# yunjinli/visual-slam

Measured on AMD Instinct MI355X. Metric: stereo frames/sec, detect+describe (1500 feats) + stereo match, 752x480, higher is better.
Workload: dtype u8/f32/f64; 1 GPU; synthetic 752x480 stereo, 1500 feats/frame (BASELINE configs[1]); independent streams per GPU (configs[3]); inputs_resident_in_hbm=True, distinct_stereo_pairs_per_gpu=1024, distinct_scenes_per_gpu=64, stereo_frames_per_pass_per_gpu=1024, hip_streams=2, stereo_frames_per_launch=512, num_features=1500, match=threshold 70, ratio 1.2, cross-check

## Files before the change

include/vslam_hip.h:

```cpp
#ifndef VSLAM_HIP_H
#define VSLAM_HIP_H

#include <stddef.h>
#include <stdint.h>

#ifdef __cplusplus
extern "C" {
#endif

#define VSL_OK 0
#define VSL_ERR_INVALID (-1)
#define VSL_ERR_HIP (-2)
#define VSL_ERR_NOMEM (-3)
#define VSL_ERR_CAPACITY (-4)
#define VSL_ERR_NO_DEVICE (-5)
#define VSL_ERR_IO (-6)
#define VSL_ERR_NUMERIC (-7)

typedef struct vsl_ctx vsl_ctx;


const char* vsl_version(void);
const char* vsl_last_error(const vsl_ctx* ctx);
int vsl_device_count(void);
// ... 74 lines not shown
int vsl_frames_upload(vsl_ctx* ctx, vsl_frames* f, int first, int n, const uint8_t* imgs,
                      size_t pitch, size_t img_stride);
int vsl_host_register(vsl_ctx* ctx, void* ptr, size_t bytes);
int vsl_host_unregister(vsl_ctx* ctx, void* ptr);
int vsl_frames_detect_describe(vsl_ctx* ctx, vsl_frames* f, int first, int n, int num_features,
                               int rotate_features);
int vsl_frames_resolve_ties(vsl_ctx* ctx, vsl_frames* f, int* n_resolved);
int vsl_frames_exact_fallbacks(const vsl_frames* f);
int vsl_ctx_set_tie_eps(vsl_ctx* ctx, double eps);
int vsl_ctx_set_diagnostic(vsl_ctx* ctx, const char* name, int value);
int vsl_ctx_get_diagnostic(vsl_ctx* ctx, const char* name, int* value);

int vsl_frames_match(vsl_ctx* ctx, vsl_frames* f, const int32_t* slot_pairs, int n_pairs,
                     int threshold, double dist_2_best);
int vsl_frames_download_keypoints(vsl_ctx* ctx, vsl_frames* f, int slot, int cap,
                                  double* corners_xy, double* angles, uint64_t* desc, int* n_out);
int vsl_frames_download_matches(vsl_ctx* ctx, vsl_frames* f, int pair, int cap_pairs,
                                int32_t* pairs, int* n_out);
int vsl_frames_download_counts(vsl_ctx* ctx, vsl_frames* f, int n_images, int32_t* n_keypoints,
                               int n_pairs, int32_t* n_matches);

int vsl_frames_stereo_inliers(vsl_ctx* ctx, vsl_frames* f, int first_pair, int n_pairs, int model_a, const double* intr8_a,
                              int model_b, const double* intr8_b, const double* E9, const double* R9_0_1,
                              const double* t3_0_1, double threshold, int triangulate);
int vsl_frames_download_inliers(vsl_ctx* ctx, vsl_frames* f, int pair, int cap_pairs, int32_t* pairs, double* points_c,
                                int* n_out);
int vsl_frames_download_inlier_counts(vsl_ctx* ctx, vsl_frames* f, int n_pairs, int32_t* counts);
int vsl_find_inliers_essential(vsl_ctx* ctx, int model_a, const double* intr8_a, int model_b, const double* intr8_b,
                               const double* E9, const double* kp_a_xy, int n_a, const double* kp_b_xy, int n_b,
                               const int32_t* matches, int n_matches, double threshold, const double* R9_0_1,
                               const double* t3_0_1, int32_t* pairs_out, double* points_out, int* n_out);

int vsl_frames_download_candidate_counts(vsl_ctx* ctx, vsl_frames* f, int n_images, int32_t* n_candidates);

int vsl_diag_sqrt_check(vsl_ctx* ctx, uint32_t lo_bits, uint32_t hi_bits, unsigned long long* n_mismatch);

int vsl_diag_frames_describe_at(vsl_ctx* ctx, vsl_frames* f, int first, int n, const int32_t* corners_xy,
                                const int32_t* counts, int cap, int rotate_features, int32_t* moments,
                                int32_t* tie_rec, int tie_rec_cap, int* n_ties);

int vsl_diag_frames_set_keypoints(vsl_ctx* ctx, vsl_frames* f, int first, int n, const int32_t* counts, int cap,
                                  const int32_t* corners_xy, const uint64_t* desc);

int vsl_map_create(vsl_ctx* ctx, int cap_landmarks, int cap_descriptors, vsl_map** out);
void vsl_map_destroy(vsl_map* map);
int vsl_map_append_descriptors(vsl_map* map, int n, const uint64_t* desc, int* first_index);
int vsl_map_append_descriptors_from_frame(vsl_map* map, vsl_frames* f, int slot, int n, const int32_t* feature_ids,
                                          int* first_index);
int vsl_map_set_landmarks(vsl_map* map, int n, const double* points, const int32_t* obs_start,
                          const int32_t* obs_pool_index);
int vsl_map_info(const vsl_map* map, int* n_landmarks, int* n_observation_refs, int* n_descriptors);
int vsl_map_track(vsl_map* map, vsl_frames* f, int slot, const double* pose7, int cam_model, const double* intr8, int width,
                  int height, double cam_z_threshold, double match_max_dist_2d, int feature_match_threshold,
                  double feature_match_dist_2_best, int32_t* pairs, int* n_pairs, int* n_projected);
int vsl_map_track_corners(vsl_map* map, vsl_frames* f, int slot, const double* pose7, int cam_model, const double* intr8,
                          int width, int height, double cam_z_threshold, double match_max_dist_2d, int feature_match_threshold,
                          double feature_match_dist_2_best, int32_t* pairs, int* n_pairs, int* n_projected, double* corners_xy,
                          int* n_corners);

enum { VSL_CAM_DS = 0, VSL_CAM_PINHOLE = 1, VSL_CAM_EUCM = 2, VSL_CAM_KB4 = 3 };

typedef struct vsl_ba_problem {
  int32_t n_cams;
  int32_t n_lms;
  int32_t n_obs;
  int32_t cam_model[2];
// ... 173 lines not shown
```

visual-slam_amd/__init__.py:

```python
import ctypes as C
import os
from pathlib import Path

import numpy as np

_DIR = Path(__file__).resolve().parent
_SO = _DIR / "libvslam_hip.so"
_LIB = None

u8p = C.POINTER(C.c_uint8)
i32p = C.POINTER(C.c_int32)
u32p = C.POINTER(C.c_uint32)
u64p = C.POINTER(C.c_uint64)
i64p = C.POINTER(C.c_int64)
f32p = C.POINTER(C.c_float)
f64p = C.POINTER(C.c_double)

STAGES = ["response", "select", "describe", "match", "match_finalize", "ba_linearize", "ba_schur",
          "ba_solve", "bow_transform", "bow_score", "ba_finish", "ba_step"]

SPD_PATHS = ["none", "dense_panels", "band_panels", "band_fused", "band_two_ended", "bcr", "bcr_cyclic"]

OK = 0
CAM_DS, CAM_PINHOLE, CAM_EUCM, CAM_KB4 = 0, 1, 2, 3
# ... 953 lines not shown

    def bow_vectors(self, first, n, voc, num_features=1500, levelsup=4, db=None, cap_per_image=None, host_outputs=True):
        L, ctx = self.ctx.L, self.ctx
        n = int(n)
        cap = (2 * num_features + 512 if cap_per_image is None else int(cap_per_image)) if host_outputs else 0
        nfeat = np.zeros(max(n, 1), np.int32)
        index = np.zeros(max(n, 1), np.int32)
        for attempt in range(2):
            m = max(n * cap, 1)
            ids, vals = np.zeros(m, np.uint32), np.zeros(m, np.float64)
            fn, ff = np.zeros(m, np.uint32), np.zeros(m, np.uint32)
            nnz, fvn = np.zeros(max(n, 1), np.int32), np.zeros(max(n, 1), np.int32)
            rc = L.vsl_frames_bow_vectors(ctx.h, self.h, int(first), n, voc.h if voc is not None else None, int(num_features),
                                          int(levelsup), db.h if db is not None else None, index.ctypes.data_as(i32p), cap,
                                          ids.ctypes.data_as(u32p), vals.ctypes.data_as(f64p), nnz.ctypes.data_as(i32p),
                                          fn.ctypes.data_as(u32p), ff.ctypes.data_as(u32p), fvn.ctypes.data_as(i32p),
                                          nfeat.ctypes.data_as(i32p))
            if rc != -4 or cap == 0 or cap_per_image is not None or nfeat[:n].max(initial=0) <= cap:
                break
            cap = int(nfeat[:n].max())
        ctx._ck(rc)
        out = None
        if host_outputs:
            out = [(ids[i * cap:i * cap + nnz[i]].copy(), vals[i * cap:i * cap + nnz[i]].copy(),
                    fn[i * cap:i * cap + fvn[i]].copy(), ff[i * cap:i * cap + fvn[i]].copy()) for i in range(n)]
        return (out, index[:n].copy()) if db is not None else out

    def candidate_counts(self, n_images):
        nc = np.zeros(max(n_images, 1), np.int32)
        self.ctx._ck(self.ctx.L.vsl_frames_download_candidate_counts(self.ctx.h, self.h, int(n_images),
                                                                     nc.ctypes.data_as(i32p)))
        return nc[:n_images].copy()

    def counts(self, n_images, n_pairs):
        nk = np.zeros(max(n_images, 1), np.int32)
        nm = np.zeros(max(n_pairs, 1), np.int32)
        self.ctx._ck(self.ctx.L.vsl_frames_download_counts(self.ctx.h, self.h, int(n_images),
                                                           nk.ctypes.data_as(i32p), int(n_pairs),
                                                           nm.ctypes.data_as(i32p)))
        return nk[:n_images].copy(), nm[:n_pairs].copy()


class Map:

    def __init__(self, ctx, cap_landmarks=4096, cap_descriptors=16384):
        self.ctx = ctx
        hnd = C.c_void_p()
        ctx._ck(ctx.L.vsl_map_create(ctx.h, int(cap_landmarks), int(cap_descriptors), C.byref(hnd)))
        self.h = hnd

    def close(self):
        if getattr(self, "h", None):
            self.ctx.L.vsl_map_destroy(self.h)
            self.h = None

    def __del__(self):
        try:
            self.close()
        except Exception:
            pass

    def append_descriptors(self, desc):
        desc = np.ascontiguousarray(desc, np.uint64).reshape(-1, 4)
        first = C.c_int32()
        self.ctx._ck(self.ctx.L.vsl_map_append_descriptors(self.h, len(desc), desc.ctypes.data_as(u64p), C.byref(first)))
        return first.value
# ... 41 lines not shown
```

visual-slam_amd/csrc/ctx.hip:

```cpp
#include <cmath>

#include "vsl_common.h"

static thread_local char g_noctx_err[512] = "";

int vsl_fail(vsl_ctx* ctx, int code, const char* fmt, ...) {
  char* dst = ctx ? ctx->err : g_noctx_err;
  va_list ap;
  va_start(ap, fmt);
  vsnprintf(dst, 512, fmt, ap);
  va_end(ap);
  return code;
}

extern "C" const char* vsl_version(void) { return "vslam_hip 0.1 (gfx950)"; }

extern "C" const char* vsl_last_error(const vsl_ctx* ctx) { return ctx ? ctx->err : g_noctx_err; }

extern "C" int vsl_device_count(void) {
  int n = 0;
  if (hipGetDeviceCount(&n) != hipSuccess) return 0;
  return n;
}

// ... 204 lines not shown
    ctx->stage_launches[i] = 0;
  }
  return rc;
}

template <class T>
static hipError_t dalloc(T** p, size_t n) {
  return hipMalloc((void**)p, n * sizeof(T));
}

int vsl_frames_alloc(vsl_ctx* ctx, int max_images, int w, int h, int F, int max_pairs, vsl_frames** out) {
  if (!ctx || !out) return VSL_ERR_INVALID;
  *out = nullptr;
  if (max_images <= 0 || w < 40 || h < 40 || w > 65535 || h > 65535 || F <= 0 || max_pairs < 0 || (int64_t)w * h >= (1ll << 31) ||
      F >= (1 << 22))
    return vsl_fail(ctx, VSL_ERR_INVALID, "vsl_frames_create: bad sizes images=%d w=%d h=%d F=%d pairs=%d", max_images, w, h, F, max_pairs);
  VSL_HIP(ctx, hipSetDevice(ctx->device));
  vsl_frames* f = new (std::nothrow) vsl_frames;
  if (!f) return vsl_fail(ctx, VSL_ERR_NOMEM, "out of host memory");
  f->device = ctx->device;
  f->max_images = max_images;
  f->w = w;
  f->h = h;
  f->F = F;
  f->max_pairs = max_pairs;
  f->cand_cap = (size_t)w * h;
  f->tie_cap = 4096;
  const size_t px = (size_t)w * h, M = (size_t)max_images, P = (size_t)(max_pairs > 0 ? max_pairs : 1);
  bool ok = true;
  ok = ok && dalloc(&f->images, M * px) == hipSuccess;
  ok = ok && dalloc(&f->response, M * px) == hipSuccess;
  ok = ok && dalloc(&f->meta, M * VSL_META_STRIDE) == hipSuccess;
  ok = ok && dalloc(&f->cand, M * f->cand_cap) == hipSuccess;
  ok = ok && dalloc(&f->kp_xy, M * F * 2) == hipSuccess;
  ok = ok && dalloc(&f->kp_count, M) == hipSuccess;
  ok = ok && dalloc(&f->kp_moments, M * F * 2) == hipSuccess;
  ok = ok && dalloc(&f->kp_angle, M * F) == hipSuccess;
  ok = ok && dalloc(&f->kp_desc, M * F * 4) == hipSuccess;
  ok = ok && dalloc(&f->pair_slots, P * 2) == hipSuccess;
  ok = ok && dalloc(&f->best_key, P * 2 * F) == hipSuccess;
  ok = ok && dalloc(&f->second_key, P * 2 * F) == hipSuccess;
  ok = ok && dalloc(&f->matches, P * F * 2) == hipSuccess;
  ok = ok && dalloc(&f->match_count, P) == hipSuccess;
  ok = ok && dalloc(&f->exact_list, M * VSL_EXACT_CAP) == hipSuccess;
  const int tiles_x = (w + (1 << VSL_TILE_LX) - 1) >> VSL_TILE_LX, tiles_y = (h + (1 << VSL_TILE_LY) - 1) >> VSL_TILE_LY;
  if (w % 16 == 0 && F < (1 << (32 - VSL_TILE_LX - VSL_TILE_LY)) && tiles_x * tiles_y <= 1024) {
    f->tiles_x = tiles_x;
    f->tiles = tiles_x * tiles_y;
    ok = ok && dalloc(&f->tile_off, M * (size_t)(f->tiles + 1)) == hipSuccess;
    ok = ok && dalloc(&f->tile_ent, M * F) == hipSuccess;
  }
  ok = ok && dalloc(&f->tie_count, 1) == hipSuccess;
  ok = ok && dalloc(&f->tie_rec, (size_t)f->tie_cap * 4) == hipSuccess;
  if (!ok) {
    vsl_frames_destroy(f);
    return vsl_fail(ctx, VSL_ERR_NOMEM, "device allocation failed for frame store (%d images %dx%d)", max_images, w, h);
  }
  (void)hipMemsetAsync(f->kp_count, 0, M * sizeof(int32_t), ctx->stream);
  (void)hipMemsetAsync(f->match_count, 0, P * sizeof(int32_t), ctx->stream);
  (void)hipMemsetAsync(f->tie_count, 0, sizeof(int32_t), ctx->stream);
  (void)hipMemsetAsync(f->meta, 0, M * VSL_META_STRIDE * sizeof(int32_t), ctx->stream);
  VSL_HIP(ctx, hipStreamSynchronize(ctx->stream));
  *out = f;
  return VSL_OK;
}

extern "C" int vsl_frames_create(vsl_ctx* ctx, int max_images, int w, int h, int max_features, int max_pairs,
                                 vsl_frames** out) {
  return vsl_frames_alloc(ctx, max_images, w, h, max_features, max_pairs, out);
}

extern "C" int vsl_frames_destroy(vsl_frames* f) {
  if (!f) return VSL_OK;
  (void)hipSetDevice(f->device);
  (void)hipDeviceSynchronize();
  void* ptrs[] = {f->images, f->response, f->meta, f->cand, f->kp_xy, f->kp_count,
                  f->kp_moments, f->kp_angle, f->kp_desc, f->pair_slots, f->best_key, f->second_key,
                  f->matches, f->match_count, f->tie_count, f->tie_rec, f->sel_grid, f->exact_list, f->tile_off, f->tile_ent,
                  f->st_pairs, f->st_points, f->st_count};
  for (void* p : ptrs)
    if (p) (void)hipFree(p);
  delete f;
  return VSL_OK;
}

extern "C" void* vsl_frames_images_dev(vsl_frames* f) { return f ? (void*)f->images : nullptr; }

extern "C" int vsl_frames_upload(vsl_ctx* ctx, vsl_frames* f, int first, int n, const uint8_t* imgs, size_t pitch,
                                 size_t img_stride) {
  if (!ctx || !f || !imgs || first < 0 || n < 0 || first + n > f->max_images || pitch < (size_t)f->w)
    return vsl_fail(ctx, VSL_ERR_INVALID, "vsl_frames_upload: bad arguments");
  if (n == 0) return VSL_OK;
  VSL_HIP(ctx, hipSetDevice(ctx->device));
  const size_t img_bytes = (size_t)f->w * f->h;
  if (pitch == (size_t)f->w && img_stride == img_bytes) {
    VSL_HIP(ctx, hipMemcpyAsync(f->images + (size_t)first * img_bytes, imgs, (size_t)n * img_bytes, hipMemcpyHostToDevice,
                                ctx->stream));
    return VSL_OK;
  }
  for (int i = 0; i < n; i++) {
    VSL_HIP(ctx, hipMemcpy2DAsync(f->images + (size_t)(first + i) * img_bytes, f->w, imgs + (size_t)i * img_stride,
                                  pitch, f->w, f->h, hipMemcpyHostToDevice, ctx->stream));
  }
  return VSL_OK;
}

extern "C" int vsl_host_register(vsl_ctx* ctx, void* ptr, size_t bytes) {
  if (!ctx || !ptr || bytes == 0) return vsl_fail(ctx, VSL_ERR_INVALID, "vsl_host_register: bad arguments");
  VSL_HIP(ctx, hipSetDevice(ctx->device));
  VSL_HIP(ctx, hipHostRegister(ptr, bytes, hipHostRegisterDefault));
  return VSL_OK;
// ... 58 lines not shown
    ctx->scratch = nullptr;
  }
  if (!ctx->scratch) {
    int rc = vsl_frames_alloc(ctx, 2, w, h, feat, 1, &ctx->scratch);
    if (rc) return rc;
    ctx->scratch_w = w;
    ctx->scratch_h = h;
    ctx->scratch_feat = feat;
  }
  *out = ctx->scratch;
  return VSL_OK;
}

extern "C" int vsl_frames_download_counts(vsl_ctx* ctx, vsl_frames* f, int n_images, int32_t* n_keypoints,
                                          int n_pairs, int32_t* n_matches) {
  if (!ctx || !f || n_images < 0 || n_images > f->max_images || n_pairs < 0 || n_pairs > f->max_pairs)
    return vsl_fail(ctx, VSL_ERR_INVALID, "vsl_frames_download_counts: bad arguments");
  if (n_images > 0 && n_keypoints)
    VSL_HIP(ctx, hipMemcpyAsync(n_keypoints, f->kp_count, sizeof(int32_t) * n_images, hipMemcpyDeviceToHost, ctx->stream));
  if (n_pairs > 0 && n_matches)
    VSL_HIP(ctx, hipMemcpyAsync(n_matches, f->match_count, sizeof(int32_t) * n_pairs, hipMemcpyDeviceToHost, ctx->stream));
  VSL_HIP(ctx, hipStreamSynchronize(ctx->stream));
  return VSL_OK;
}

extern "C" int vsl_frames_download_candidate_counts(vsl_ctx* ctx, vsl_frames* f, int n_images, int32_t* n_candidates) {
  if (!ctx || !f || n_images < 0 || n_images > f->max_images || !n_candidates)
    return vsl_fail(ctx, VSL_ERR_INVALID, "vsl_frames_download_candidate_counts: bad arguments");
  if (n_images == 0) return VSL_OK;
  std::vector<int32_t> m((size_t)n_images * VSL_META_STRIDE);
  VSL_HIP(ctx, hipMemcpyAsync(m.data(), f->meta, sizeof(int32_t) * m.size(), hipMemcpyDeviceToHost, ctx->stream));
  VSL_HIP(ctx, hipStreamSynchronize(ctx->stream));
  for (int i = 0; i < n_images; i++) n_candidates[i] = m[(size_t)i * VSL_META_STRIDE + VSL_META_NCAND_LAST];
  return VSL_OK;
}

extern "C" int vsl_frames_download_keypoints(vsl_ctx* ctx, vsl_frames* f, int slot, int cap, double* corners_xy,
                                             double* angles, uint64_t* desc, int* n_out) {
  if (!ctx || !f || slot < 0 || slot >= f->max_images || !n_out || cap < 0)
    return vsl_fail(ctx, VSL_ERR_INVALID, "vsl_frames_download_keypoints: bad arguments");
  const size_t F = (size_t)f->F;
  void* hp = nullptr;
  int rc = vsl_ctx_hpinned(ctx, 64 + F * (8 + 8 + 32), &hp);
  if (rc) return rc;
  int32_t* hdr = (int32_t*)hp;
  int32_t* hxy = (int32_t*)((char*)hp + 64);
  int32_t* hmom = hxy + 2 * F;
  uint64_t* hdesc = (uint64_t*)(hmom + 2 * F);
  const size_t base = (size_t)slot * F;
  const bool ties = f->ties_pending;
  hdr[0] = 0;
  if (ties) VSL_HIP(ctx, hipMemcpyAsync(&hdr[0], f->tie_count, sizeof(int32_t), hipMemcpyDeviceToHost, ctx->stream));
  VSL_HIP(ctx, hipMemcpyAsync(&hdr[1], f->kp_count + slot, sizeof(int32_t), hipMemcpyDeviceToHost, ctx->stream));
  VSL_HIP(ctx, hipMemcpyAsync(hxy, f->kp_xy + base * 2, sizeof(int32_t) * 2 * F, hipMemcpyDeviceToHost, ctx->stream));
  if (angles) VSL_HIP(ctx, hipMemcpyAsync(hmom, f->kp_moments + base * 2, sizeof(int32_t) * 2 * F, hipMemcpyDeviceToHost, ctx->stream));
  if (desc) VSL_HIP(ctx, hipMemcpyAsync(hdesc, f->kp_desc + base * 4, sizeof(uint64_t) * 4 * F, hipMemcpyDeviceToHost, ctx->stream));
  VSL_HIP(ctx, hipStreamSynchronize(ctx->stream));
  if (ties) {
    if (hdr[0] != 0) {
      if ((rc = vsl_resolve_ties(ctx, f, nullptr))) return rc;
      if (desc) {
        VSL_HIP(ctx, hipMemcpyAsync(hdesc, f->kp_desc + base * 4, sizeof(uint64_t) * 4 * F, hipMemcpyDeviceToHost, ctx->stream));
        VSL_HIP(ctx, hipStreamSynchronize(ctx->stream));
      }
    } else {
      f->ties_settled();
// ... 62 lines not shown
```

visual-slam_amd/csrc/detect.hip:

```cpp
#include <type_traits>

#include "vsl_common.h"

#ifndef K1_ROWS
#define K1_ROWS 60
#endif
#ifndef K1_ROWS_SMALL
#define K1_ROWS_SMALL 29
#endif
#define VSL_QUALITY_LEVEL 0.01
#define K1_WLIST 384
#define K1_COLS 60

__device__ __forceinline__ int reflect101(int i, int n) { return i < 0 ? -i : (i >= n ? 2 * n - 2 - i : i); }

struct RowF {
  float rx, ry;
};

struct RowRaw {
  unsigned l, m, r;
};

typedef __amdgpu_buffer_rsrc_t ImgSrd;
// ... 407 lines not shown
      const int b = top >= LOGK - 1 ? top - (LOGK - 1) : 0;
      const int nb = top - b + 1;
#pragma unroll 1
      for (int tid = tid0; tid < REPS * SEL_THREADS; tid += SEL_THREADS) {
      const int t_hi = tid >> b, t_lo = tid & ((1 << b) - 1);
      const int i0 = (t_hi << (b + LOGK)) | t_lo;
      uint64_t rk[KPT];
#pragma unroll
      for (int r = 0; r < KPT; r++) rk[r] = keys[SEL_PHYS(i0 | (r << b))];
#pragma unroll
      for (int x = LOGK - 1; x >= 0; x--) {
        if (x < nb) {
#pragma unroll
          for (int r = 0; r < KPT; r++) {
            if ((r & (1 << x)) == 0) {
              const bool desc = ((i0 | (r << b)) & k) == 0;
              const uint64_t u = rk[r], v = rk[r | (1 << x)];
              const bool sw = desc ? (u < v) : (u > v);
              rk[r] = sw ? v : u;
              rk[r | (1 << x)] = sw ? u : v;
            }
          }
        }
      }
#pragma unroll
      for (int r = 0; r < KPT; r++) keys[SEL_PHYS(i0 | (r << b))] = rk[r];
      }
      __syncthreads();
      top = b - 1;
    }
  }
}

template <bool GRID_GLOBAL>
__global__ __launch_bounds__(SEL_THREADS) void select_kernel(const uint64_t* __restrict__ cand_all,
                                                             int32_t* meta,
                                                             int32_t* __restrict__ kp_xy, int32_t* __restrict__ kp_count,
                                                             int w, int h, size_t cand_cap, int F, int first,
                                                             int num_features, int border, double quality,
                                                             uint32_t* __restrict__ grid_scratch, int bucket_cap) {
  __shared__ __align__(16) unsigned char smem[SEL_LDS_BYTES];
  const int slot = first + blockIdx.x;
  const uint64_t* __restrict__ cand = cand_all + (size_t)slot * cand_cap;
  const int n_cand_raw = meta[(size_t)slot * VSL_META_STRIDE + VSL_META_NCAND];
  const int n_cand = min(n_cand_raw, (int)cand_cap);
  const int gw = (w + 7) / 8 + 2, gh = (h + 7) / 8 + 2, cells = (gw * gh + 1) & ~1;
  uint64_t* keys = (uint64_t*)smem;
  uint32_t* keys32 = (uint32_t*)smem;
  SelShared* sh = (SelShared*)(smem + SEL_KEYS_PADDED * 8);
  int* next = (int*)(smem + SEL_KEYS_PADDED * 8 + 2048);
  typedef typename SelGrid<GRID_GLOBAL>::u16 grid_u16;
  typedef typename SelGrid<GRID_GLOBAL>::u32 grid_u32;
  grid_u16* acc = GRID_GLOBAL ? (grid_u16*)(grid_scratch + (size_t)slot * cells) : (grid_u16*)(next + 3 * SEL_THREADS);
  grid_u16* head = acc + cells;
  unsigned long long* node = (unsigned long long*)next;
  int* state = next + 2 * SEL_THREADS;
  const int tid = threadIdx.x;

  int n_acc = 0, n_out = 0;
  unsigned long long hi = ~0ull;
  int32_t* out = kp_xy + (size_t)slot * F * 2;
  const float maxv = vsl_ordered_to_float(meta[(size_t)slot * VSL_META_STRIDE + VSL_META_MAX]);
  const float thr = (float)((double)maxv * quality);
  const unsigned long long floor_key =
      (((unsigned long long)((uint32_t)vsl_float_to_ordered(thr) ^ 0x80000000u)) << 32) | 0xFFFFFFFFull;
  int remaining = 0;
  int* bcount = next;
  int* bstart = next + SEL_THREADS;
  int* bcursor = next + 2 * SEL_THREADS;
  uint32_t* stage = (uint32_t*)bcursor;
  static_assert(SEL_BINS == SEL_THREADS, "one bin per thread");
  const uint32_t hi_max = (uint32_t)vsl_float_to_ordered(maxv) ^ 0x80000000u;
  const uint32_t hi_floor = (uint32_t)vsl_float_to_ordered(thr) ^ 0x80000000u;
  int bshift = 16;
  while (bshift < 31 && (hi_max >> bshift) - (hi_floor >> bshift) >= (uint32_t)SEL_BINS) bshift++;
  const uint32_t bin_top = hi_max >> bshift;
  bool bucket_sort = false;
  const bool in_regs = n_cand <= SEL_CHUNK;
  unsigned long long rk[SEL_KPT] = {};
  if (maxv > 0.f) {
    bcount[tid] = 0;
    if (tid == 0) sh->n_chunk = 0;
    __syncthreads();
    if (in_regs) {
#pragma unroll
      for (int k = 0; k < SEL_KPT; k++) {
        const int i = tid + k * SEL_THREADS;
        rk[k] = i < n_cand ? cand[i] : 0ull;
      }
#pragma unroll
      for (int k = 0; k < SEL_KPT; k++)
        if (rk[k] > floor_key) atomicAdd(&bcount[bin_top - min((uint32_t)(rk[k] >> 32) >> bshift, bin_top)], 1);
    } else {
      for (int i = tid; i < n_cand; i += SEL_THREADS) {
        const unsigned long long key = cand[i];
        if (key > floor_key) {
          const uint32_t kb = min((uint32_t)(key >> 32) >> bshift, bin_top);
          atomicAdd(&bcount[bin_top - kb], 1);
        }
      }
    }
    __syncthreads();
    const int c = bcount[tid];
    int x = c;
    const int lane = tid & 63, wv = tid >> 6;
#pragma unroll
    for (int o = 1; o < 64; o <<= 1) {
      const int y = __shfl_up(x, o);
      if (lane >= o) x += y;
    }
    int cmax = c;
#pragma unroll
    for (int o = 32; o > 0; o >>= 1) cmax = max(cmax, __shfl_xor(cmax, o));
// ... 48 lines not shown
        pos_off = SEL_POS_UPPER;
      } else {
#pragma unroll
        for (int k = 0; k < SEL_KPT; k++)
          if ((uint32_t)(rk[k] >> 32) < (uint32_t)SEL_CHUNK) keys32[(uint32_t)(rk[k] >> 32)] = (uint32_t)rk[k];
        __syncthreads();
      }
    } else {
      for (int i = tid; i < n_cand; i += SEL_THREADS) {
        const unsigned long long key = cand[i];
        if (key > floor_key) {
          const int bin = (int)(bin_top - min((uint32_t)(key >> 32) >> bshift, bin_top));
          const int p = bstart[bin] + atomicAdd(&bcursor[bin], 1);
          keys[SEL_PHYS(p)] = key;
        }
      }
      __syncthreads();
      for (int p = tid; p < remaining; p += SEL_THREADS) {
        const unsigned long long key = keys[SEL_PHYS(p)];
        const int bin = (int)(bin_top - min((uint32_t)(key >> 32) >> bshift, bin_top));
        const int s0 = bstart[bin], e0 = s0 + bcount[bin];
        int larger = 0;
        for (int q = s0; q < e0; q++) larger += keys[SEL_PHYS(q)] > key;
        stage[s0 + larger] = (uint32_t)key;
      }
      __syncthreads();
      for (int p = tid; p < remaining; p += SEL_THREADS) keys32[p] = stage[p];
      __syncthreads();
      for (int i = tid; i < cells; i += SEL_THREADS) ((grid_u32*)acc)[i] = i < (cells >> 1) ? 0u : ~0u;
      __syncthreads();
    }
    compact = true;
  }

  while (remaining > 0 && n_acc < num_features) {
    unsigned long long lo = 0;
    if (remaining > SEL_CHUNK) {
      unsigned long long prefix = 0;
      int k = SEL_CHUNK;
      for (int shift = 56; shift >= 0; shift -= 8) {
        for (int i = tid; i < 256; i += SEL_THREADS) sh->hist[i] = 0;
        __syncthreads();
        const unsigned long long pmask = shift == 56 ? 0ull : (~0ull << (shift + 8));
        for (int i = tid; i < n_cand; i += SEL_THREADS) {
          const unsigned long long key = cand[i];
          if (key < hi && key > floor_key && (key & pmask) == prefix) atomicAdd(&sh->hist[(int)((key >> shift) & 255)], 1);
        }
        __syncthreads();
        if (tid == 0) {
          int kk = k, d = 255;
          for (; d > 0; d--) {
            if (sh->hist[d] >= kk) break;
            kk -= sh->hist[d];
          }
          sh->sel_k = kk;
          sh->sel_prefix = prefix | ((unsigned long long)d << shift);
        }
        __syncthreads();
        k = sh->sel_k;
        prefix = sh->sel_prefix;
        __syncthreads();
      }
      lo = prefix;
    }
    int n_chunk;
    if (compact) {
// ... 11 lines not shown
      __syncthreads();
      n_chunk = min(sh->n_chunk, SEL_CHUNK);
      int N = 1024;
      while (N < n_chunk) N <<= 1;
      for (int i = n_chunk + tid; i < N; i += SEL_THREADS) keys[SEL_PHYS(i)] = 0ull;
      __syncthreads();
      if (N >= 2048) {
        if (N == 8192) sel_sort_blocked<2, 2>(keys, tid, 13);
        else if (N == 4096) sel_sort_blocked<2, 1>(keys, tid, 12);
        else sel_sort_blocked<1, 1>(keys, tid, 11);
      } else {
        for (int k = 2; k <= N; k <<= 1) {
          for (int j = k >> 1; j > 0; j >>= 1) {
            for (int t = tid; t < (N >> 1); t += SEL_THREADS) {
              const int i = ((t & ~(j - 1)) << 1) | (t & (j - 1));
              const int l = i | j;
              const uint64_t a = keys[SEL_PHYS(i)], b = keys[SEL_PHYS(l)];
              const bool desc = (i & k) == 0;
              if (desc ? (a < b) : (a > b)) {
                keys[SEL_PHYS(i)] = b;
                keys[SEL_PHYS(l)] = a;
              }
            }
            __syncthreads();
          }
        }
      }
    }
    for (int r0 = 0; r0 < n_chunk && n_acc < num_features; r0 += SEL_THREADS) {
      const int r = r0 + tid;
      int px = 0, py = 0, cell = 0;
      bool alive = false;
      if (r < n_chunk) {
        const uint32_t pix = compact ? keys32[pos_off + r] :(uint32_t)(keys[SEL_PHYS(r)] & 0xFFFFFFFFull);
        py = (int)(pix >> 16);
        px = (int)(pix & 0xFFFFu);
        cell = ((py >> 3) + 1) * gw + (px >> 3) + 1;
        const int lx = px & 7, ly = py & 7;
        int near = 0;
#pragma unroll
        for (int oy = -1; oy <= 1; oy++) {
          const int row = cell + oy * gw;
          const uint32_t t0 = acc[row - 1], t1 = acc[row], t2 = acc[row + 1];
#pragma unroll
          for (int k = 0; k < 6; k++) {
            const uint32_t b = ((k >> 1) == 0 ? t0 : (k >> 1) == 1 ? t1 : t2) >> (8 * (k & 1));
            const int dx = lx - 8 * ((k >> 1) - 1) - (int)(b & 7u), dy = ly - 8 * oy - (int)((b >> 3) & 7u);
            const unsigned d2 = (unsigned)(dx * dx) + (unsigned)(dy * dy);
            near |= (int)((b & SEL_ACC_VALID) != 0u) & (int)(d2 < 64u);
          }
        }
        alive = near == 0;
      }
      state[tid] = alive ? 0 : 2;
      {
        const uint32_t prev = alive ? sel_xchg16(head, cell, (uint32_t)tid) : SEL_HEAD_EMPTY;
        const int nxt = sel_head_rank(prev);
        node[tid] = ((unsigned long long)(uint32_t)nxt << 32) | ((uint32_t)px | ((uint32_t)py << 16));
      }
      __syncthreads();
      int nb = 0;
      unsigned long long blk = 0ull;
      if (alive) {
#pragma unroll 1
        for (int oy = -1; oy <= 1; oy++) {
          const int row = cell + oy * gw;
          uint32_t h3[3];
#pragma unroll
          for (int k = 0; k < 3; k++) h3[k] = head[row + k - 1];
#pragma unroll
          for (int k = 0; k < 3; k++)
            for (int u = sel_head_rank(h3[k]); u >= 0;) {
              const unsigned long long nd = node[u];
              const int uu = u;
              u = (int)(nd >> 32);
              if (uu < tid) {
                const uint32_t q = (uint32_t)nd;
                const int dx = px - (int)(q & 0xFFFF), dy = py - (int)(q >> 16);
                if (dx * dx + dy * dy < 64) {
                  blk = (blk << 10) | (unsigned long long)(unsigned)uu;
                  nb++;
                }
              }
            }
        }
      }
      bool undecided = alive, accepted = false;
      while (__ballot(undecided) != 0ull) {
        if (undecided) {
          bool rej = false, blocked = false;
          if (nb <= SEL_MAX_BLOCKERS) {
#pragma unroll
// ... 78 lines not shown
  if (num_features < 1 || num_features > f->F)
    return vsl_fail(ctx, VSL_ERR_INVALID, "num_features %d not in [1, %d]", num_features, f->F);
  static_assert(sizeof(SelShared) <= 2048, "SelShared fits its LDS slot");
  const int cells = (((f->w + 7) / 8 + 2) * ((f->h + 7) / 8 + 2) + 1) & ~1;
  const bool grid_global = cells > SEL_MAX_CELLS;
  if (grid_global && !f->sel_grid) {
    VSL_HIP(ctx, hipMalloc((void**)&f->sel_grid, sizeof(uint32_t) * (size_t)cells * f->max_images));
  }
  const int w = f->w, h = f->h;
  {
    VslStage st(ctx, VSL_STAGE_RESPONSE);
    if (f->detect_meta_dirty)
      hipLaunchKernelGGL(detect_init_kernel, dim3((f->max_images + 255) / 256), dim3(256), 0, ctx->stream, f->meta, 0, f->max_images);
    f->detect_meta_dirty = true;
    const bool small = n < 8 && !f->store_response;
    const int rows = small ? K1_ROWS_SMALL : K1_ROWS;
    const int tiles_y = (h + 4 * rows - 1) / (4 * rows);
    const int tiles_x = (w + K1_COLS - 1) / K1_COLS;
    const dim3 k1_grid((unsigned)(tiles_x * tiles_y) * (unsigned)(n >= 8 ? 8 * ((n + 7) / 8) : n));
    const int wcap = ctx->k1_list_cap < 0 ? K1_WLIST : min(ctx->k1_list_cap, K1_WLIST);
    if (f->store_response)
      hipLaunchKernelGGL((min_eig_response_kernel<true, K1_ROWS>), k1_grid, dim3(256), 0, ctx->stream, f->images, f->response, f->meta,
                         f->cand, f->cand_cap, w, h, first, wcap, n, tiles_x, tiles_y);
    else if (small)
      hipLaunchKernelGGL((min_eig_response_kernel<false, K1_ROWS_SMALL>), k1_grid, dim3(256), 0, ctx->stream, f->images, f->response, f->meta,
                         f->cand, f->cand_cap, w, h, first, wcap, n, tiles_x, tiles_y);
    else
      hipLaunchKernelGGL((min_eig_response_kernel<false, K1_ROWS>), k1_grid, dim3(256), 0, ctx->stream, f->images, f->response, f->meta,
                         f->cand, f->cand_cap, w, h, first, wcap, n, tiles_x, tiles_y);
    VSL_CHECK_LAUNCH(ctx);
  }
  {
    VslStage st(ctx, VSL_STAGE_SELECT);
    if (grid_global)
      hipLaunchKernelGGL(select_kernel<true>, dim3(n), dim3(SEL_THREADS), 0, ctx->stream, f->cand, f->meta, f->kp_xy,
                         f->kp_count, w, h, f->cand_cap, f->F, first, num_features, 19, VSL_QUALITY_LEVEL, f->sel_grid, ctx->select_bucket_cap);
    else
      hipLaunchKernelGGL(select_kernel<false>, dim3(n), dim3(SEL_THREADS), 0, ctx->stream, f->cand, f->meta, f->kp_xy,
                         f->kp_count, w, h, f->cand_cap, f->F, first, num_features, 19, VSL_QUALITY_LEVEL, (uint32_t*)nullptr,
                         ctx->select_bucket_cap);
    VSL_CHECK_LAUNCH(ctx);
  }
  f->detect_meta_dirty = false;
  return VSL_OK;
}
```

visual-slam_amd/csrc/keypoints_api.hip:

```cpp
#include <cmath>
#include <string>

#include "vsl_common.h"

extern "C" int vsl_ctx_set_tie_eps(vsl_ctx* ctx, double eps) {
  if (!ctx || !(eps >= 0.0) || eps > 0.5) return vsl_fail(ctx, VSL_ERR_INVALID, "tie eps must be in [0, 0.5]");
  ctx->tie_eps = eps;
  return VSL_OK;
}

extern "C" int vsl_ctx_set_diagnostic(vsl_ctx* ctx, const char* name, int value) {
  if (!ctx || !name) return VSL_ERR_INVALID;
  const std::string k(name);
  if (k == "match_use_valu") ctx->match_use_valu = value != 0;
  else if (k == "match_no_stagger") ctx->match_no_stagger = value != 0;
  else if (k == "match_use_i8") ctx->match_use_i8 = value != 0;
  else if (k == "force_generic_describe") ctx->force_generic_describe = value != 0;
  else if (k == "describe_tile_min_images") ctx->describe_tile_min_images = value;
  else if (k == "bow_keys64") ctx->bow_keys64 = value != 0;
  else if (k == "match_two_pass") ctx->match_two_pass = value != 0;
  else if (k == "k1_list_cap") ctx->k1_list_cap = value;
  else if (k == "exact_list_cap") ctx->exact_list_cap = value;
  else if (k == "vo_chain_ticket") ctx->vo_chain_ticket = value;
  else if (k == "pending_desc_max") ctx->pending_desc_max = value < 1 ? 1 : value;
  else if (k == "ba_schur_entries") ctx->ba_schur_entries = value != 0;
  else if (k == "bow_no_wg_score") ctx->bow_no_wg_score = value != 0;
  else if (k == "ba_no_fused") ctx->ba_no_fused = value != 0;
  else if (k == "ba_host_lm") ctx->ba_host_lm = value != 0;
  else if (k == "ba_no_cyclic") ctx->ba_no_cyclic = value != 0;
  else if (k == "ba_schur_atomics") ctx->ba_schur_atomics = value != 0;
  else if (k == "ba_iterative_schur") ctx->ba_iterative_schur = value != 0;
  else if (k == "ba_pcg_poll") ctx->ba_pcg_poll = value < 0 ? 0 : value;
  else if (k == "ba_pcg_tol_exp") ctx->ba_pcg_tol_exp = value < 0 ? 0 : value;
  else if (k == "ba_force_dense") ctx->ba_force_dense = value != 0;
  else if (k == "pgo_cov_no_band_read") ctx->pgo_cov_no_band_read = value != 0;
  else if (k == "ba_cov_no_band_read") ctx->ba_cov_no_band_read = value != 0;
  else if (k == "pgo_far_edges") ctx->pgo_far_edges = value != 0;
  else if (k == "chol_no_fused")ctx->chol_no_fused = value != 0;
  else if (k == "chol_no_bcr") ctx->chol_no_bcr = value != 0;
  else if (k == "chol_one_ended") ctx->chol_one_ended = value != 0;
  else if (k == "frames_bow_chunk") ctx->frames_bow_chunk = value < 0 ? 0 : value;
  else if (k == "select_bucket_cap") ctx->select_bucket_cap = value < 0 ? 0 : value;
  else return vsl_fail(ctx, VSL_ERR_INVALID, "vsl_ctx_set_diagnostic: unknown knob '%s'", name);
  return VSL_OK;
}

extern "C" int vsl_ctx_get_diagnostic(vsl_ctx* ctx, const char* name, int* value) {
  if (!ctx || !name || !value) return VSL_ERR_INVALID;
  const std::string k(name);
  if (k == "ba_iterative_schur") *value = ctx->ba_iterative_schur ? 1 : 0;
  else if (k == "ba_pcg_poll") *value = ctx->ba_pcg_poll;
  else if (k == "ba_pcg_tol_exp") *value = ctx->ba_pcg_tol_exp;
  else if (k == "pgo_far_edges") *value = ctx->pgo_far_edges ? 1 : 0;
  else return vsl_fail(ctx, VSL_ERR_INVALID, "vsl_ctx_get_diagnostic: knob '%s' cannot be read back", name);
  return VSL_OK;
}

extern "C" int vsl_frames_detect_describe(vsl_ctx* ctx, vsl_frames* f, int first, int n, int num_features,
                                          int rotate_features) {
  if (!ctx || !f || first < 0 || n < 0 || first + n > f->max_images)
    return vsl_fail(ctx, VSL_ERR_INVALID, "vsl_frames_detect_describe: bad slot range [%d, %d)", first, first + n);
  VSL_HIP(ctx, hipSetDevice(ctx->device));
  int rc = vsl_launch_detect(ctx, f, first, n, num_features);
  if (rc) return rc;
  return vsl_launch_describe(ctx, f, first, n, rotate_features, 0);
}

extern "C" int vsl_frames_resolve_ties(vsl_ctx* ctx, vsl_frames* f, int* n_resolved) {
  if (!ctx || !f) return VSL_ERR_INVALID;
  VSL_HIP(ctx, hipSetDevice(ctx->device));
  return vsl_resolve_ties(ctx, f, n_resolved);
}

extern "C" int vsl_frames_exact_fallbacks(const vsl_frames* f) {
  return f ? f->exact_fallbacks : VSL_ERR_INVALID;
// ... 161 lines not shown
```

visual-slam_amd/csrc/vsl_common.h:

```cpp
#pragma once
#include <hip/hip_runtime.h>

#include <chrono>
#include <cstdarg>
#include <cstdint>
#include <cstdio>
#include <cstring>
#include <string>
#include <vector>

#include "../../include/vslam_hip.h"
#include "chol_plan.h"

#define VSL_WAVE 64
#define VSL_META_STRIDE 32
#define VSL_META_MAX 0
#define VSL_META_NCAND 1
#define VSL_META_NEXACT 3
#define VSL_META_NCAND_LAST 4
#define VSL_META_NEXACT_LAST 5
#define VSL_EXACT_CAP 16384
#ifndef VSL_TILE_LX
#define VSL_TILE_LX 7
#endif
#ifndef VSL_TILE_LY
#define VSL_TILE_LY 7
#endif
#define VSL_TIE_OVERFLOW_FLAG 0x40000000u

inline double now_ms() {
  return std::chrono::duration<double, std::milli>(std::chrono::steady_clock::now().time_since_epoch()).count();
}

struct vsl_ctx {
  int device = 0;
  hipStream_t stream = nullptr;
  bool owns_stream = false;
  char err[512] = {0};
  bool profiling = false;
  struct StageEv {
    hipEvent_t a, b;
    int stage;
  };
  std::vector<StageEv> pending;
  std::vector<hipEvent_t> ev_pool;
  double stage_ms[VSL_STAGE_COUNT] = {0};
  int64_t stage_launches[VSL_STAGE_COUNT] = {0};
  struct vsl_frames* scratch = nullptr;
  int scratch_w = 0, scratch_h = 0, scratch_feat = 0;
  void* dscratch = nullptr;
  size_t dscratch_cap = 0;
  void* hpinned = nullptr;
  size_t hpinned_cap = 0;
// ... 14 lines not shown
  bool bow_query_attr_set = false;
  double* status_word = nullptr;
  double tie_eps = 1e-12;
  bool match_use_i8 = false;
  bool match_no_stagger = false;
  bool match_two_pass = false;
  bool match_use_valu = false;
  bool force_generic_describe = false;
  int select_bucket_cap = 128;
  bool chol_no_bcr = false;
  bool chol_one_ended = false;
  bool chol_no_fused = false;
  bool ba_force_dense = false;
  bool pgo_cov_no_band_read = false;
  bool ba_cov_no_band_read = false;
  bool pgo_far_edges = false;
  int last_pgo_far_taken = 0, last_pgo_far_k = 0, last_pgo_far_bw = 0, last_pgo_far_cols = 0;
  int64_t last_pgo_far_solves = 0;
  bool ba_schur_atomics = false;
  bool ba_no_fused = false;
  bool ba_schur_entries = false;
  int describe_tile_min_images = 96;
  bool ba_iterative_schur = false;
  int ba_pcg_poll = 0;
  int ba_pcg_tol_exp = 0;
  bool ba_no_cyclic = false;
  bool ba_host_lm = false;
  bool bow_no_wg_score = false;
  bool bow_keys64 = false;
  int vo_chain_ticket = 0;
  int pending_desc_max = 64;
  int exact_list_cap = VSL_EXACT_CAP;
  int frames_bow_chunk = 0;
  int k1_list_cap = -1;
};

int vsl_fail(vsl_ctx* ctx, int code, const char* fmt, ...);

int vsl_ba_fused_solve(vsl_ctx* ctx, const vsl_ba_problem* prob, const vsl_ba_options* opt, vsl_ba_summary* summary, int* handled);
int vsl_ba_chol_small_launch(vsl_ctx* ctx, int n, const double* S, const double* rhs, double* dc, int* ok_flag);

#define VSL_HIP(ctx, call)                                                                        \
  do {                                                                                            \
    hipError_t e_ = (call);                                                                       \
    if (e_ != hipSuccess)                                                                         \
      return vsl_fail((ctx), VSL_ERR_HIP, "%s:%d %s -> %s", __FILE__, __LINE__, #call,            \
                      hipGetErrorString(e_));                                                     \
  } while (0)

#define VSL_CHECK_LAUNCH(ctx)                                                                     \
  do {                                                                                            \
    hipError_t e_ = hipGetLastError();                                                            \
    if (e_ != hipSuccess)                                                                         \
      return vsl_fail((ctx), VSL_ERR_HIP, "%s:%d kernel launch -> %s", __FILE__, __LINE__,        \
                      hipGetErrorString(e_));                                                     \
  } while (0)

int vsl_ctx_dscratch(vsl_ctx* ctx, size_t bytes, void** out);
int vsl_ctx_hpinned(vsl_ctx* ctx, size_t bytes, void** out);

struct VslStage {
  vsl_ctx* ctx;
  int idx = -1;
  VslStage(vsl_ctx* c, int stage);
  ~VslStage();
};

struct vsl_frames {
  int device = 0;
  int max_images = 0, w = 0, h = 0, F = 0, max_pairs = 0;
  size_t cand_cap = 0;
  uint8_t* images = nullptr;
  float* response = nullptr;
  int32_t* meta = nullptr;
  uint64_t* cand = nullptr;
  int32_t* kp_xy = nullptr;
  int32_t* kp_count = nullptr;
  int32_t* kp_moments = nullptr;
  double* kp_angle = nullptr;
  uint64_t* kp_desc = nullptr;
  int32_t* pair_slots = nullptr;
  uint32_t* best_key = nullptr;
  uint32_t* second_key = nullptr;
  int32_t* matches = nullptr;
  int32_t* match_count = nullptr;
  uint32_t* exact_list = nullptr;
  int32_t* tile_off = nullptr;
  uint32_t* tile_ent = nullptr;
  int tiles_x = 0, tiles = 0;
  uint32_t* sel_grid = nullptr;
  int32_t* tie_count = nullptr;
  int32_t* tie_rec = nullptr;
  int tie_cap = 0;
  bool ties_pending = false, ties_from_angles = false;
  bool detect_meta_dirty = true;
  bool describe_meta_dirty = true;
  struct DescRange {
    int first, n, rotate;
  };
  std::vector<DescRange> pending_desc;
  void ties_settled() {
    ties_pending = false;
    pending_desc.clear();
  }
  int exact_fallbacks = 0;
  bool store_response = false;
  std::vector<int32_t> pair_cache;
  int32_t* st_pairs = nullptr;
  double* st_points = nullptr;
  int32_t* st_count = nullptr;
  std::vector<uint8_t> st_has_points;
};

int vsl_frames_alloc(vsl_ctx* ctx, int max_images, int w, int h, int F, int max_pairs, vsl_frames** out);

int vsl_launch_detect(vsl_ctx* ctx, vsl_frames* f, int first, int n, int num_features);
int vsl_launch_describe(vsl_ctx* ctx, vsl_frames* f, int first, int n, int rotate_features,
                        int from_angles);
int vsl_launch_match(vsl_ctx* ctx, vsl_frames* f, int n_pairs, int threshold, double dist_2_best, int db_bound);
int vsl_resolve_ties(vsl_ctx* ctx, vsl_frames* f, int* n_resolved);
int vsl_set_pairs(vsl_ctx* ctx, vsl_frames* f, const int32_t* slot_pairs, int n_pairs);

// ... 76 lines not shown
```

Before: 383,300 frames/s.

## Add rank pre-pass kernel that counting-sorts candidates before grid selection

Adds a separate rank_candidates kernel that counting-sorts each image's above-threshold corner candidates into a fully ordered pixel-position array in global memory, using 16-bit packed LDS bin counters and an in-bucket rank. The select kernel then skips its own bucket/chunk sorting and streams positions from that array, prefetching the next chunk's entry. The aim is to pull the sort out of the LDS-heavy select kernel into a lighter, higher-occupancy kernel. The cost is an extra launch, an extra global buffer and a write/read round trip, with a fallback to the old path when candidates overflow the cap or a bucket exceeds bucket_cap.

Measured after the change: 386,000 frames/s (median of 6 runs). About the same (+0.7%).

```diff
diff --git a/include/vslam_hip.h b/include/vslam_hip.h
--- a/include/vslam_hip.h
+++ b/include/vslam_hip.h
@@ -130,6 +130,8 @@
                                const double* t3_0_1, int32_t* pairs_out, double* points_out, int* n_out);
 
 int vsl_frames_download_candidate_counts(vsl_ctx* ctx, vsl_frames* f, int n_images, int32_t* n_candidates);
+
+int vsl_frames_download_ranked_counts(vsl_ctx* ctx, vsl_frames* f, int n_images, int32_t* n_ranked);
 
 int vsl_diag_sqrt_check(vsl_ctx* ctx, uint32_t lo_bits, uint32_t hi_bits, unsigned long long* n_mismatch);
 
diff --git a/visual-slam_amd/__init__.py b/visual-slam_amd/__init__.py
--- a/visual-slam_amd/__init__.py
+++ b/visual-slam_amd/__init__.py
@@ -1009,6 +1009,12 @@
                                                                      nc.ctypes.data_as(i32p)))
         return nc[:n_images].copy()
 
+    def ranked_counts(self, n_images):
+        nr = np.zeros(max(n_images, 1), np.int32)
+        self.ctx._ck(self.ctx.L.vsl_frames_download_ranked_counts(self.ctx.h, self.h, int(n_images),
+                                                                  nr.ctypes.data_as(i32p)))
+        return nr[:n_images].copy()
+
     def counts(self, n_images, n_pairs):
         nk = np.zeros(max(n_images, 1), np.int32)
         nm = np.zeros(max(n_pairs, 1), np.int32)
diff --git a/visual-slam_amd/csrc/ctx.hip b/visual-slam_amd/csrc/ctx.hip
--- a/visual-slam_amd/csrc/ctx.hip
+++ b/visual-slam_amd/csrc/ctx.hip
@@ -260,6 +260,7 @@
   ok = ok && dalloc(&f->response, M * px) == hipSuccess;
   ok = ok && dalloc(&f->meta, M * VSL_META_STRIDE) == hipSuccess;
   ok = ok && dalloc(&f->cand, M * f->cand_cap) == hipSuccess;
+  ok = ok && dalloc(&f->rank_pos, M * VSL_RANK_CAP) == hipSuccess;
   ok = ok && dalloc(&f->kp_xy, M * F * 2) == hipSuccess;
   ok = ok && dalloc(&f->kp_count, M) == hipSuccess;
   ok = ok && dalloc(&f->kp_moments, M * F * 2) == hipSuccess;
@@ -304,7 +305,7 @@
   (void)hipDeviceSynchronize();
   void* ptrs[] = {f->images, f->response, f->meta, f->cand, f->kp_xy, f->kp_count,
                   f->kp_moments, f->kp_angle, f->kp_desc, f->pair_slots, f->best_key, f->second_key,
-                  f->matches, f->match_count, f->tie_count, f->tie_rec, f->sel_grid, f->exact_list, f->tile_off, f->tile_ent,
+                  f->matches, f->match_count, f->tie_count, f->tie_rec, f->sel_grid, f->rank_pos, f->exact_list, f->tile_off, f->tile_ent,
                   f->st_pairs, f->st_points, f->st_count};
   for (void* p : ptrs)
     if (p) (void)hipFree(p);
@@ -429,6 +430,17 @@
   VSL_HIP(ctx, hipMemcpyAsync(m.data(), f->meta, sizeof(int32_t) * m.size(), hipMemcpyDeviceToHost, ctx->stream));
   VSL_HIP(ctx, hipStreamSynchronize(ctx->stream));
   for (int i = 0; i < n_images; i++) n_candidates[i] = m[(size_t)i * VSL_META_STRIDE + VSL_META_NCAND_LAST];
+  return VSL_OK;
+}
+
+extern "C" int vsl_frames_download_ranked_counts(vsl_ctx* ctx, vsl_frames* f, int n_images, int32_t* n_ranked) {
+  if (!ctx || !f || n_images < 0 || n_images > f->max_images || !n_ranked)
+    return vsl_fail(ctx, VSL_ERR_INVALID, "vsl_frames_download_ranked_counts: bad arguments");
+  if (n_images == 0) return VSL_OK;
+  std::vector<int32_t> m((size_t)n_images * VSL_META_STRIDE);
+  VSL_HIP(ctx, hipMemcpyAsync(m.data(), f->meta, sizeof(int32_t) * m.size(), hipMemcpyDeviceToHost, ctx->stream));
+  VSL_HIP(ctx, hipStreamSynchronize(ctx->stream));
+  for (int i = 0; i < n_images; i++) n_ranked[i] = m[(size_t)i * VSL_META_STRIDE + VSL_META_NRANKED];
   return VSL_OK;
 }
 
diff --git a/visual-slam_amd/csrc/detect.hip b/visual-slam_amd/csrc/detect.hip
--- a/visual-slam_amd/csrc/detect.hip
+++ b/visual-slam_amd/csrc/detect.hip
@@ -463,13 +463,175 @@
   }
 }
 
+struct SelBins {
+  unsigned long long floor_key;
+  uint32_t bin_top;
+  int bshift;
+};
+__device__ __forceinline__ SelBins sel_bins(float maxv, double quality) {
+  const float thr = (float)((double)maxv * quality);
+  const uint32_t hi_max = (uint32_t)vsl_float_to_ordered(maxv) ^ 0x80000000u;
+  const uint32_t hi_floor = (uint32_t)vsl_float_to_ordered(thr) ^ 0x80000000u;
+  SelBins b;
+  b.floor_key = ((unsigned long long)hi_floor << 32) | 0xFFFFFFFFull;
+  b.bshift = 16;
+  while (b.bshift < 31 && (hi_max >> b.bshift) - (hi_floor >> b.bshift) >= (uint32_t)SEL_BINS) b.bshift++;
+  b.bin_top = hi_max >> b.bshift;
+  return b;
+}
+
+#define RANK_CAP_NARROW 4592
+static_assert(VSL_RANK_CAP == SEL_CHUNK, "the position array holds whatever the counting sort accepts");
+template <int THREADS, int CAP, int FINE>
+__global__ __launch_bounds__(THREADS) void rank_candidates_kernel(const uint64_t* __restrict__ cand_all, int32_t* meta,
+                                                                  uint32_t* __restrict__ rank_pos, size_t cand_cap,
+                                                                  int first, double quality, int bucket_cap) {
+  constexpr int BINS = SEL_BINS << FINE, KPT = (CAP + THREADS - 1) / THREADS, BPT = BINS / THREADS, WAVES = THREADS / 64;
+  static_assert(BINS % THREADS == 0 && BPT % 2 == 0 && BPT % (1 << FINE) == 0, "a thread's bins of the prefix are whole words and whole response bins");
+  static_assert(CAP <= VSL_RANK_CAP && CAP < 65536, "a slot index fits a u16 and the position array");
+  __shared__ __align__(16) unsigned char smem[CAP * 8 + BINS * 2 + 128];
+  static_assert((THREADS == 256 ? 4 : 2) * sizeof(smem) <= 160 * 1024, "pre-pass workgroups per CU");
+  uint64_t* keys = (uint64_t*)smem;
+  uint32_t* binw = (uint32_t*)(smem + CAP * 8);
+  int* wtot = (int*)(smem + CAP * 8 + BINS * 2);
+  static_assert((2 * WAVES + 1) * 4 <= 128, "scan scratch");
+  const int slot = first + blockIdx.x, tid = threadIdx.x, lane = tid & 63, wv = tid >> 6;
+  int32_t* m = meta + (size_t)slot * VSL_META_STRIDE;
+  const uint64_t* __restrict__ cand = cand_all + (size_t)slot * cand_cap;
+  const int n_cand = min(m[VSL_META_NCAND], (int)cand_cap);
+  const float maxv = vsl_ordered_to_float(m[VSL_META_MAX]);
+  if (!(maxv > 0.f)) {
+    if (tid == 0) m[VSL_META_NRANKED] = 0;
+    return;
+  }
+  const SelBins sb = sel_bins(maxv, quality);
+  const unsigned long long floor_key = sb.floor_key;
+  const int fshift = sb.bshift - FINE;
+  const uint32_t fine_top = (sb.bin_top << FINE) | ((1u << FINE) - 1u);
+#define RANK_FBIN(key) ((int)(fine_top - min((uint32_t)((key) >> 32) >> fshift, fine_top)))
+  for (int i = tid; i < BINS / 2; i += THREADS) binw[i] = 0u;
+  if (tid == 0) wtot[2 * WAVES] = 0;
+  __syncthreads();
+  const bool in_regs = n_cand <= CAP;
+  unsigned long long rk[KPT] = {};
+  int mine = 0;
+  if (in_regs) {
+#pragma unroll
+    for (int k = 0; k < KPT; k++) {
+      const int i = tid + k * THREADS;
+      rk[k] = i < n_cand ? cand[i] : 0ull;
+    }
+#pragma unroll
+    for (int k = 0; k < KPT; k++)
+      if (rk[k] > floor_key) {
+        const int fb = RANK_FBIN(rk[k]);
+        atomicAdd(&binw[fb >> 1], 1u << ((fb & 1) * 16));
+        mine++;
+      }
+  } else {
+    for (int i = tid; i < n_cand; i += THREADS) {
+      const unsigned long long key = cand[i];
+      if (key > floor_key) {
+        const int fb = RANK_FBIN(key);
+        atomicAdd(&binw[fb >> 1], 1u << ((fb & 1) * 16));
+        mine++;
+      }
+    }
+  }
+#pragma unroll
+  for (int o = 32; o > 0; o >>= 1) mine += __shfl_xor(mine, o);
+  if (lane == 0) atomicAdd(&wtot[2 * WAVES], mine);
+  __syncthreads();
+  const int remaining = wtot[2 * WAVES];
+  if (remaining == 0 || remaining > CAP) {
+    if (tid == 0) m[VSL_META_NRANKED] = remaining == 0 ? 0 : -1;
+    return;
+  }
+  int c[BPT];
+#pragma unroll
+  for (int j = 0; j < BPT / 2; j++) {
+    const uint32_t w2 = binw[tid * (BPT / 2) + j];
+    c[2 * j] = (int)(w2 & 0xFFFFu);
+    c[2 * j + 1] = (int)(w2 >> 16);
+  }
+  int sum = 0, fullest = 0;
+#pragma unroll
+  for (int g = 0; g < (BPT >> FINE); g++) {
+    int cs = 0;
+#pragma unroll
+    for (int j = 0; j < (1 << FINE); j++) cs += c[(g << FINE) + j];
+    fullest = max(fullest, cs);
+    sum += cs;
+  }
+  int x = sum;
+#pragma unroll
+  for (int o = 1; o < 64; o <<= 1) {
+    const int y = __shfl_up(x, o);
+    if (lane >= o) x += y;
+  }
+#pragma unroll
+  for (int o = 32; o > 0; o >>= 1) fullest = max(fullest, __shfl_xor(fullest, o));
+  if (lane == 63) wtot[wv] = x;
+  if (lane == 0) wtot[WAVES + wv] = fullest;
+  __syncthreads();
+  int s = x - sum;
+#pragma unroll
+  for (int k = 0; k < WAVES; k++) {
+    s += k < wv ? wtot[k] : 0;
+    fullest = max(fullest, wtot[WAVES + k]);
+  }
+  if (fullest > bucket_cap) {
+    if (tid == 0) m[VSL_META_NRANKED] = -1;
+    return;
+  }
+#pragma unroll
+  for (int j = 0; j < BPT / 2; j++) {
+    const uint32_t s0 = (uint32_t)s, s1 = (uint32_t)(s + c[2 * j]);
+    s += c[2 * j] + c[2 * j + 1];
+    binw[tid * (BPT / 2) + j] = s0 | (s1 << 16);
+  }
+  __syncthreads();
+  if (in_regs) {
+#pragma unroll
+    for (int k = 0; k < KPT; k++)
+      if (rk[k] > floor_key) {
+        const int fb = RANK_FBIN(rk[k]), sh16 = (fb & 1) * 16;
+        const uint32_t p = (atomicAdd(&binw[fb >> 1], 1u << sh16) >> sh16) & 0xFFFFu;
+        keys[p] = rk[k];
+      }
+  } else {
+    for (int i = tid; i < n_cand; i += THREADS) {
+      const unsigned long long key = cand[i];
+      if (key > floor_key) {
+        const int fb = RANK_FBIN(key), sh16 = (fb & 1) * 16;
+        const uint32_t p = (atomicAdd(&binw[fb >> 1], 1u << sh16) >> sh16) & 0xFFFFu;
+        keys[p] = key;
+      }
+    }
+  }
+  __syncthreads();
+  const uint16_t* bend = (const uint16_t*)binw;
+  uint32_t* __restrict__ out = rank_pos + (size_t)slot * VSL_RANK_CAP;
+  for (int p = tid; p < remaining; p += THREADS) {
+    const unsigned long long key = keys[p];
+    const int fb = RANK_FBIN(key);
+    const int e0 = bend[fb], s0 = fb ? bend[fb - 1] : 0;
+    int larger = 0;
+    for (int q = s0; q < e0; q++) larger += keys[q] > key;
+    out[s0 + larger] = (uint32_t)key;
+  }
+#undef RANK_FBIN
+  if (tid == 0) m[VSL_META_NRANKED] = remaining;
+}
+
 template <bool GRID_GLOBAL>
 __global__ __launch_bounds__(SEL_THREADS) void select_kernel(const uint64_t* __restrict__ cand_all,
                                                              int32_t* meta,
                                                              int32_t* __restrict__ kp_xy, int32_t* __restrict__ kp_count,
                                                              int w, int h, size_t cand_cap, int F, int first,
                                                              int num_features, int border, double quality,
-                                                             uint32_t* __restrict__ grid_scratch, int bucket_cap) {
+                                                             uint32_t* __restrict__ grid_scratch, int bucket_cap,
+                                                             const uint32_t* __restrict__ rank_pos) {
   __shared__ __align__(16) unsigned char smem[SEL_LDS_BYTES];
   const int slot = first + blockIdx.x;
   const uint64_t* __restrict__ cand = cand_all + (size_t)slot * cand_cap;
@@ -491,25 +653,24 @@
   int n_acc = 0, n_out = 0;
   unsigned long long hi = ~0ull;
   int32_t* out = kp_xy + (size_t)slot * F * 2;
+  const int n_ranked = rank_pos ? meta[(size_t)slot * VSL_META_STRIDE + VSL_META_NRANKED] : -1;
+  const bool ranked = n_ranked >= 0;
+  const uint32_t* __restrict__ rpos = rank_pos + (size_t)slot * VSL_RANK_CAP;
   const float maxv = vsl_ordered_to_float(meta[(size_t)slot * VSL_META_STRIDE + VSL_META_MAX]);
-  const float thr = (float)((double)maxv * quality);
-  const unsigned long long floor_key =
-      (((unsigned long long)((uint32_t)vsl_float_to_ordered(thr) ^ 0x80000000u)) << 32) | 0xFFFFFFFFull;
+  const SelBins sb = sel_bins(maxv, quality);
+  const unsigned long long floor_key = sb.floor_key;
   int remaining = 0;
   int* bcount = next;
   int* bstart = next + SEL_THREADS;
   int* bcursor = next + 2 * SEL_THREADS;
   uint32_t* stage = (uint32_t*)bcursor;
   static_assert(SEL_BINS == SEL_THREADS, "one bin per thread");
-  const uint32_t hi_max = (uint32_t)vsl_float_to_ordered(maxv) ^ 0x80000000u;
-  const uint32_t hi_floor = (uint32_t)vsl_float_to_ordered(thr) ^ 0x80000000u;
-  int bshift = 16;
-  while (bshift < 31 && (hi_max >> bshift) - (hi_floor >> bshift) >= (uint32_t)SEL_BINS) bshift++;
-  const uint32_t bin_top = hi_max >> bshift;
+  const int bshift = sb.bshift;
+  const uint32_t bin_top = sb.bin_top;
   bool bucket_sort = false;
   const bool in_regs = n_cand <= SEL_CHUNK;
   unsigned long long rk[SEL_KPT] = {};
-  if (maxv > 0.f) {
+  if (!ranked && maxv > 0.f) {
     bcount[tid] = 0;
     if (tid == 0) sh->n_chunk = 0;
     __syncthreads();
@@ -624,6 +785,11 @@
     }
     compact = true;
   }
+  if (ranked) {
+    remaining = n_ranked;
+    compact = true;
+  }
+  uint32_t pix_next = ranked && tid < n_ranked ? rpos[tid] : 0u;
 
   while (remaining > 0 && n_acc < num_features) {
     unsigned long long lo = 0;
@@ -701,7 +867,7 @@
       int px = 0, py = 0, cell = 0;
       bool alive = false;
       if (r < n_chunk) {
-        const uint32_t pix = compact ? keys32[pos_off + r] :(uint32_t)(keys[SEL_PHYS(r)] & 0xFFFFFFFFull);
+        const uint32_t pix = ranked ? pix_next : compact ? keys32[pos_off + r] : (uint32_t)(keys[SEL_PHYS(r)] & 0xFFFFFFFFull);
         py = (int)(pix >> 16);
         px = (int)(pix & 0xFFFFu);
         cell = ((py >> 3) + 1) * gw + (px >> 3) + 1;
@@ -727,6 +893,7 @@
         const int nxt = sel_head_rank(prev);
         node[tid] = ((unsigned long long)(uint32_t)nxt << 32) | ((uint32_t)px | ((uint32_t)py << 16));
       }
+      if (ranked && r + SEL_THREADS < n_chunk) pix_next = rpos[r + SEL_THREADS];
       __syncthreads();
       int nb = 0;
       unsigned long long blk = 0ull;
@@ -871,13 +1038,25 @@
   }
   {
     VslStage st(ctx, VSL_STAGE_SELECT);
+    const bool prepass = ctx->select_prepass_min > 0 && n >= ctx->select_prepass_min;
+    if (prepass) {
+      if (ctx->select_prepass_wide)
+        hipLaunchKernelGGL((rank_candidates_kernel<512, SEL_CHUNK, 2>), dim3(n), dim3(512), 0, ctx->stream, f->cand, f->meta,
+                           f->rank_pos, f->cand_cap, first, VSL_QUALITY_LEVEL, ctx->select_bucket_cap);
+      else
+        hipLaunchKernelGGL((rank_candidates_kernel<256, RANK_CAP_NARROW, 1>), dim3(n), dim3(256), 0, ctx->stream, f->cand, f->meta,
+                           f->rank_pos, f->cand_cap, first, VSL_QUALITY_LEVEL, ctx->select_bucket_cap);
+      VSL_CHECK_LAUNCH(ctx);
+    }
+    const uint32_t* rank_pos = prepass ? f->rank_pos : nullptr;
     if (grid_global)
       hipLaunchKernelGGL(select_kernel<true>, dim3(n), dim3(SEL_THREADS), 0, ctx->stream, f->cand, f->meta, f->kp_xy,
-                         f->kp_count, w, h, f->cand_cap, f->F, first, num_features, 19, VSL_QUALITY_LEVEL, f->sel_grid, ctx->select_bucket_cap);
+                         f->kp_count, w, h, f->cand_cap, f->F, first, num_features, 19, VSL_QUALITY_LEVEL, f->sel_grid,
+                         ctx->select_bucket_cap, rank_pos);
     else
       hipLaunchKernelGGL(select_kernel<false>, dim3(n), dim3(SEL_THREADS), 0, ctx->stream, f->cand, f->meta, f->kp_xy,
                          f->kp_count, w, h, f->cand_cap, f->F, first, num_features, 19, VSL_QUALITY_LEVEL, (uint32_t*)nullptr,
-                         ctx->select_bucket_cap);
+                         ctx->select_bucket_cap, rank_pos);
     VSL_CHECK_LAUNCH(ctx);
   }
   f->detect_meta_dirty = false;
diff --git a/visual-slam_amd/csrc/keypoints_api.hip b/visual-slam_amd/csrc/keypoints_api.hip
--- a/visual-slam_amd/csrc/keypoints_api.hip
+++ b/visual-slam_amd/csrc/keypoints_api.hip
@@ -41,6 +41,8 @@
   else if (k == "chol_one_ended") ctx->chol_one_ended = value != 0;
   else if (k == "frames_bow_chunk") ctx->frames_bow_chunk = value < 0 ? 0 : value;
   else if (k == "select_bucket_cap") ctx->select_bucket_cap = value < 0 ? 0 : value;
+  else if (k == "select_prepass_min") ctx->select_prepass_min = value < 0 ? 0 : value;
+  else if (k == "select_prepass_wide") ctx->select_prepass_wide = value != 0;
   else return vsl_fail(ctx, VSL_ERR_INVALID, "vsl_ctx_set_diagnostic: unknown knob '%s'", name);
   return VSL_OK;
 }
diff --git a/visual-slam_amd/csrc/vsl_common.h b/visual-slam_amd/csrc/vsl_common.h
--- a/visual-slam_amd/csrc/vsl_common.h
+++ b/visual-slam_amd/csrc/vsl_common.h
@@ -19,6 +19,8 @@
 #define VSL_META_NEXACT 3
 #define VSL_META_NCAND_LAST 4
 #define VSL_META_NEXACT_LAST 5
+#define VSL_META_NRANKED 6
+#define VSL_RANK_CAP 8192
 #define VSL_EXACT_CAP 16384
 #ifndef VSL_TILE_LX
 #define VSL_TILE_LX 7
@@ -99,6 +101,8 @@
   int pending_desc_max = 64;
   int exact_list_cap = VSL_EXACT_CAP;
   int frames_bow_chunk = 0;
+  int select_prepass_min = 8;
+  bool select_prepass_wide = false;
   int k1_list_cap = -1;
 };
 
@@ -155,6 +159,7 @@
   int32_t* tile_off = nullptr;
   uint32_t* tile_ent = nullptr;
   int tiles_x = 0, tiles = 0;
+  uint32_t* rank_pos = nullptr;
   uint32_t* sel_grid = nullptr;
   int32_t* tie_count = nullptr;
   int32_t* tie_rec = nullptr;
```
